# smileyenot983/reconstructor

Measured on AMD Instinct MI355X. Metric: descriptor pair-distances/s + BA LM-iterations/s (1k cams, 100k pts), higher is better.
Workload: dtype f16+f64

## Files before the change

reconstructor_amd/csrc/coarse_i8.h:

```cpp
#pragma once

typedef int i32x16 __attribute__((ext_vector_type(16)));
typedef int i32x4 __attribute__((ext_vector_type(4)));


__device__ __forceinline__ unsigned neg_i8x4(unsigned w)
{
    const unsigned x = ~w;
    return ((x & 0x7F7F7F7Fu) + 0x01010101u) ^ (x & 0x80808080u);
}

template <int ABL, int SH>
__global__ __launch_bounds__(512, 2) void k_coarse_top2_i8(CoarseArgs a)
{
    constexpr int ROWB = 256;
    constexpr int NCB = SH ? 4 : 2;
    constexpr int CW = SH ? 16 : 32;
    constexpr int NKS = SH ? 4 : 8;
    constexpr int CPK = SH ? 4 : 2;
    constexpr int BT = RCN_I8_BT;
    constexpr int TILEB = BT * ROWB;
    constexpr int PIECE = 64 * 16;
    constexpr int NINST = TILEB / 8 / PIECE;
    constexpr int HNP = BT / 64;
    constexpr int NG = NINST + HNP;
    constexpr int BUFB = TILEB + 8 * BT * 4;
    extern __shared__ __attribute__((aligned(16))) char smem[];

    if (!a.sc->coarse_i8) return;
    const int b = blockIdx.x;
    const int item = (b & 7) * a.items_per_xcd + (b >> 3);
    if (item >= a.n_groups * a.tiles_per_pair) return;
    const int grp = item / a.tiles_per_pair, qt = item - grp * a.tiles_per_pair;
    const int2 g = a.groups[grp];
    const int p0 = g.x, R = g.y;
    if (R == 0) return;
    const ImgDev qi = a.imgs[a.pairs[2 * p0]];
    if (qt * RCN_QT >= qi.K) return;

    const int tid = threadIdx.x, lane = tid & 63;
    const int r = SH ? (lane & 15) : (lane & 31), h = SH ? (lane >> 4) : (lane >> 5);
    const int w = __builtin_amdgcn_readfirstlane(tid >> 6);

    i32x4 bq[NCB][NKS];
#pragma unroll
    for (int cb = 0; cb < NCB; ++cb) {
        const int qrow = qt * RCN_QT + w * 64 + cb * CW + r;
        const char *base = reinterpret_cast<const char *>(qi.f16) + (size_t)qrow * ROWB;
        const int sw = qrow & 15;
#pragma unroll
        for (int ks = 0; ks < NKS; ++ks) {
            uint4 v = *reinterpret_cast<const uint4 *>(base + (((ks * CPK + h) ^ sw) << 4));
            v.x = neg_i8x4(v.x); v.y = neg_i8x4(v.y); v.z = neg_i8x4(v.z); v.w = neg_i8x4(v.w);
            bq[cb][ks] = __builtin_bit_cast(i32x4, v);
        }
    }

    struct TrainRec { const char *img; const int *hn; int nT; int pad; };
    static_assert(sizeof(TrainRec) * RCN_GROUP <= RCN_TBL_BYTES, "train-record table does not fit its LDS slot");
    TrainRec *tbl = reinterpret_cast<TrainRec *>(smem + RCN_NBUF * BUFB);
    if (tid < R) {
        const ImgDev ti = a.imgs[a.pairs[2 * (p0 + tid) + 1]];
        TrainRec rec;
        rec.img = reinterpret_cast<const char *>(ti.f16);
        rec.hn = reinterpret_cast<const int *>(ti.hn);
        rec.nT = ti.K >= 2 ? (ti.K + BT - 1) / BT : 0;
        rec.pad = 0;
        tbl[tid] = rec;
    }
    __syncthreads();
    auto tiles_of = [&](int rr) -> int { return __builtin_amdgcn_readfirstlane(tbl[rr].nT); };

    int s_pair = 0, s_tile = 0, s_nT = 0, staged = 0;
    const char *s_timg = nullptr;
    const int *s_hn = nullptr;
    auto s_seek = [&]() {
        while (s_pair < R) {
            s_nT = tiles_of(s_pair);
            if (s_nT > 0) {
                const unsigned long long pf = reinterpret_cast<unsigned long long>(tbl[s_pair].img);
                const unsigned long long ph = reinterpret_cast<unsigned long long>(tbl[s_pair].hn);
                s_timg = reinterpret_cast<const char *>(((unsigned long long)__builtin_amdgcn_readfirstlane((unsigned)(pf >> 32)) << 32) |
                                                        (unsigned)__builtin_amdgcn_readfirstlane((unsigned)pf));
                s_hn = reinterpret_cast<const int *>(((unsigned long long)__builtin_amdgcn_readfirstlane((unsigned)(ph >> 32)) << 32) |
                                                     (unsigned)__builtin_amdgcn_readfirstlane((unsigned)ph));
                s_tile = 0;
                return;
            }
            ++s_pair;
        }
    };
    auto stage_next = [&]() {
        if (s_pair >= R) return;
        char *bbase = smem + (staged % RCN_NBUF) * BUFB;
#pragma unroll
        for (int i = 0; i < NINST; ++i) {
            const int off = (w * NINST + i) * PIECE;
            const char *src = s_timg + (size_t)s_tile * TILEB + off + lane * 16;
            __builtin_amdgcn_global_load_lds(
                (const __attribute__((address_space(1))) void *)src,
                (__attribute__((address_space(3))) void *)(bbase + off), 16, 0, 0);
        }
#pragma unroll
        for (int hp = 0; hp < HNP; ++hp)
            __builtin_amdgcn_global_load_lds(
                (const __attribute__((address_space(1))) void *)(s_hn + s_tile * BT + 64 * hp + lane),
                (__attribute__((address_space(3))) void *)(bbase + TILEB + w * (BT * 4) + 256 * hp), 4, 0, 0);
        ++staged;
        if (++s_tile == s_nT) { ++s_pair; s_seek(); }
    };
    s_seek();
#pragma unroll
    for (int i = 0; i < RCN_PD; ++i) stage_next();

    unsigned m1[NCB], m2[NCB];
    i32x16 pX0, pX1, pY0, pY1;
    i32x4 qX[2][4], qY[2][4];
    auto top2 = [&](int cb, unsigned u) {
        if constexpr ((ABL & 1) != 0) return;
        const unsigned lo = min(m1[cb], m2[cb]), hi = max(m1[cb], m2[cb]);
        m2[cb] = max(lo, min(hi, u));
        m1[cb] = min(m1[cb], u);
    };
    constexpr bool LATE = ((ABL & 32) != 0) != (SH == 0);
    unsigned fk[NCB][3], fs[NCB];
    auto push = [&](int cb, int j, unsigned u) {
        if constexpr ((ABL & 1) != 0) return;
        if constexpr ((ABL & 16) != 0) { top2(cb, u); return; }
        if constexpr (LATE) {
            if ((j & 3) < 3) fk[cb][j & 3] = u;
            else top2_fold4(m1[cb], m2[cb], fk[cb][0], fk[cb][1], fk[cb][2], u);
            return;
        }
        switch (j & 3) {
        case 0: case 2: fk[cb][0] = u; break;
        case 1: fs[cb] = top2_fold_pair(m1[cb], fk[cb][0], u); break;
        default: m2[cb] = umin3(m2[cb], fs[cb], top2_fold_pair(m1[cb], fk[cb][0], u)); break;
        }
    };
    auto key = [&](int acc, unsigned idx) -> unsigned { return ((unsigned)acc << RCN_I8_IDX_BITS) | idx; };
    auto lds_read = [&](unsigned addr) -> u32x4 {
        u32x4 v;
        asm volatile("ds_read_b128 %0, %1" : "=v"(v) : "v"(addr));
        return v;
    };
    auto step = [&](i32x16 &c0, i32x16 &c1, const i32x16 &p0v, const i32x16 &p1v, unsigned tile,
                    unsigned hnl, int rb, unsigned prev_rowbase) {
        if constexpr (SH == 0) {
        const int lrow = rb * 32 + r;
        const unsigned arow = tile + lrow * ROWB;
        const int sw = lrow & 15;
        u32x4 h0, h1, h2, h3, f0, f1;
        h0 = lds_read(hnl + (rb * 32 + 0 + 4 * h) * 4);
        h1 = lds_read(hnl + (rb * 32 + 8 + 4 * h) * 4);
        h2 = lds_read(hnl + (rb * 32 + 16 + 4 * h) * 4);
        h3 = lds_read(hnl + (rb * 32 + 24 + 4 * h) * 4);
        f0 = lds_read(arow + ((h ^ sw) << 4));
        asm volatile("s_waitcnt lgkmcnt(0)" : "+v"(h0), "+v"(h1), "+v"(h2), "+v"(h3), "+v"(f0));
        i32x16 hnv;
        hnv[0] = (int)h0.x; hnv[1] = (int)h0.y; hnv[2] = (int)h0.z; hnv[3] = (int)h0.w;
        hnv[4] = (int)h1.x; hnv[5] = (int)h1.y; hnv[6] = (int)h1.z; hnv[7] = (int)h1.w;
        hnv[8] = (int)h2.x; hnv[9] = (int)h2.y; hnv[10] = (int)h2.z; hnv[11] = (int)h2.w;
        hnv[12] = (int)h3.x; hnv[13] = (int)h3.y; hnv[14] = (int)h3.z; hnv[15] = (int)h3.w;
        auto kstep = [&](int ks, u32x4 &cur, u32x4 &nxt) {
            if (ks > 0) asm volatile("s_waitcnt lgkmcnt(0)" : "+v"(cur), "+v"(c1));
            if (ks + 1 < NKS) nxt = lds_read(arow + ((((ks + 1) * 2 + h) ^ sw) << 4));
            const i32x4 av = __builtin_bit_cast(i32x4, cur);
            c0 = __builtin_amdgcn_mfma_i32_32x32x32_i8(av, bq[0][ks], ks == 0 ? hnv : c0, 0, 0, 0);
#pragma unroll
            for (int reg = ks * 16 / NKS; reg < (ks + 1) * 16 / NKS; ++reg)
                push(0, reg, key(p0v[reg], prev_rowbase + (reg & 3) + 8 * (reg >> 2)));
            c1 = __builtin_amdgcn_mfma_i32_32x32x32_i8(av, bq[1][ks], ks == 0 ? hnv : c1, 0, 0, 0);
#pragma unroll
            for (int reg = ks * 16 / NKS; reg < (ks + 1) * 16 / NKS; ++reg)
                push(1, reg, key(p1v[reg], prev_rowbase + (reg & 3) + 8 * (reg >> 2)));
        };
#pragma unroll
        for (int ks = 0; ks < NKS; ks += 2) {
            kstep(ks, f0, f1);
            kstep(ks + 1, f1, f0);
        }
        }
    };
    auto step16 = [&](i32x4 (&c)[2][4], const i32x4 (&pv)[2][4], unsigned tile, unsigned hnl, int rb, unsigned prev_rowbase) {
        if constexpr (SH == 1) {
            const int lrow = rb * 32 + r;
            const unsigned arow0 = tile + lrow * ROWB, arow1 = arow0 + 16 * ROWB;
            const int sw = lrow & 15;
            u32x4 hA, hB, f0a, f0b, f1a, f1b;
            hA = lds_read(hnl + (rb * 32 + 0 + 4 * h) * 4);
            hB = lds_read(hnl + (rb * 32 + 16 + 4 * h) * 4);
            f0a = lds_read(arow0 + ((h ^ sw) << 4));
            f0b = lds_read(arow1 + ((h ^ sw) << 4));
            asm volatile("s_waitcnt lgkmcnt(0)" : "+v"(hA), "+v"(hB), "+v"(f0a), "+v"(f0b));
            i32x4 hn[2];
            hn[0] = __builtin_bit_cast(i32x4, hA);
            hn[1] = __builtin_bit_cast(i32x4, hB);
            constexpr int EPK = 32 / NKS;
            auto kstep = [&](int ks, u32x4 &ca_, u32x4 &cb_, u32x4 &na_, u32x4 &nb_) {
                if (ks > 0) asm volatile("s_waitcnt lgkmcnt(0)" : "+v"(ca_), "+v"(cb_), "+v"(c[1][3]));
                if (ks + 1 < NKS) {
                    na_ = lds_read(arow0 + ((((ks + 1) * 4 + h) ^ sw) << 4));
                    nb_ = lds_read(arow1 + ((((ks + 1) * 4 + h) ^ sw) << 4));
                }
                const i32x4 av[2] = {__builtin_bit_cast(i32x4, ca_), __builtin_bit_cast(i32x4, cb_)};
#pragma unroll
                for (int m = 0; m < 8; ++m) {
                    const int sh = m >> 2, cb = m & 3;
                    c[sh][cb] = __builtin_amdgcn_mfma_i32_16x16x64_i8(av[sh], bq[cb][ks], ks == 0 ? hn[sh] : c[sh][cb], 0, 0, 0);
#pragma unroll
                    for (int e = ks * EPK + m * EPK / 8; e < ks * EPK + (m + 1) * EPK / 8; ++e) {
                        const int es = e >> 4, ecb = (e >> 2) & 3, er = e & 3;
                        push(ecb, er, key(pv[es][ecb][er], prev_rowbase + 16 * es + er));
                    }
                }
            };
#pragma unroll
            for (int ks = 0; ks < NKS; ks += 2) {
                kstep(ks, f0a, f0b, f1a, f1b);
                kstep(ks + 1, f1a, f1b, f0a, f0b);
            }
        }
    };
    const unsigned smem_base = (unsigned)(size_t)(const __attribute__((address_space(3))) char *)smem;

    int done = 0;
    for (int rr = 0; rr < R; ++rr) {
        const int nT = tiles_of(rr);
        if (nT == 0) continue;
#pragma unroll
        for (int cb = 0; cb < NCB; ++cb) m1[cb] = m2[cb] = 0xFFFFFFFFu;
        if constexpr (SH == 0) {
#pragma unroll
            for (int i = 0; i < 16; ++i) { pY0[i] = RCN_I8_PAD_ACC; pY1[i] = RCN_I8_PAD_ACC; }
        } else {
#pragma unroll
            for (int i = 0; i < 32; ++i) qY[i >> 4][(i >> 2) & 3][i & 3] = RCN_I8_PAD_ACC;
        }
        for (int t = 0; t < nT; ++t, ++done) {
            stage_next();
            const int ahead = staged - done - 1;
            if (ahead >= 2) asm volatile("s_waitcnt vmcnt(%0)" ::"i"(2 * NG) : "memory");
            else if (ahead == 1) asm volatile("s_waitcnt vmcnt(%0)" ::"i"(NG) : "memory");
            else asm volatile("s_waitcnt vmcnt(0)" ::: "memory");
            __builtin_amdgcn_s_barrier();
            const unsigned tile = smem_base + (done % RCN_NBUF) * BUFB;
            const unsigned hnl = tile + TILEB + w * (BT * 4);
            const unsigned base = (unsigned)(t * BT);
#pragma unroll
            for (int rb = 0; rb < BT / 32; rb += 2) {
                if constexpr (SH == 0) {
                    step(pX0, pX1, pY0, pY1, tile, hnl, rb, base + 32u * rb - 32u);
                    step(pY0, pY1, pX0, pX1, tile, hnl, rb + 1, base + 32u * rb);
                } else {
                    step16(qX, qY, tile, hnl, rb, base + 32u * rb - 32u);
                    step16(qY, qX, tile, hnl, rb + 1, base + 32u * rb);
                }
            }
        }
        if (ABL & 1) {
            if constexpr (SH == 0) asm volatile("" ::"v"(pY0), "v"(pY1), "v"(pX0), "v"(pX1));
            else {
#pragma unroll
                for (int i = 0; i < 8; ++i) asm volatile("" ::"v"(qY[i >> 2][i & 3]), "v"(qX[i >> 2][i & 3]));
            }
        }
        {
            const unsigned rowbase = (unsigned)((nT - 1) * BT + BT - 32);
            if constexpr (SH == 0) {
#pragma unroll
                for (int reg = 0; reg < 16; ++reg) {
                    const unsigned idx = rowbase + (reg & 3) + 8 * (reg >> 2);
                    push(0, reg, key(pY0[reg], idx));
                    push(1, reg, key(pY1[reg], idx));
                }
            } else {
#pragma unroll
                for (int e = 0; e < 32; ++e) {
                    const int es = e >> 4, ecb = (e >> 2) & 3, er = e & 3;
                    push(ecb, er, key(qY[es][ecb][er], rowbase + 16 * es + er));
                }
            }
        }
        if constexpr (SH == 0) {
#pragma unroll
            for (int cb = 0; cb < 2; ++cb) {
                unsigned a1 = m1[cb] | (unsigned)(4 * h), a2 = m2[cb] | (unsigned)(4 * h);
                if (m1[cb] == 0xFFFFFFFFu) a1 = 0xFFFFFFFFu;
                if (m2[cb] == 0xFFFFFFFFu) a2 = 0xFFFFFFFFu;
                unsigned b1 = __shfl_xor(a1, 32), b2 = __shfl_xor(a2, 32);
                unsigned r1 = min(a1, b1);
                unsigned r2 = min(max(a1, b1), min(a2, b2));
                const int qrow = qt * RCN_QT + w * 64 + cb * 32 + r;
                if (h == 0 && qrow < qi.K) a.cand[(size_t)(p0 + rr) * a.kq_stride + qrow] = make_uint2(r1, r2);
            }
        } else {
#pragma unroll
            for (int cb = 0; cb < 4; ++cb) {
                unsigned a1 = m1[cb] | (unsigned)(4 * h), a2 = m2[cb] | (unsigned)(4 * h);
                if (m1[cb] == 0xFFFFFFFFu) a1 = 0xFFFFFFFFu;
                if (m2[cb] == 0xFFFFFFFFu) a2 = 0xFFFFFFFFu;
#pragma unroll
                for (int o = 16; o <= 32; o <<= 1) {
                    const unsigned b1 = __shfl_xor(a1, o), b2 = __shfl_xor(a2, o);
                    const unsigned r1 = min(a1, b1);
                    a2 = min(max(a1, b1), min(a2, b2));
                    a1 = r1;
                }
                const int qrow = qt * RCN_QT + w * 64 + cb * 16 + r;
                if (h == 0 && qrow < qi.K) a.cand[(size_t)(p0 + rr) * a.kq_stride + qrow] = make_uint2(a1, a2);
            }
        }
    }
}
```

reconstructor_amd/csrc/match.hip:

```cpp
#include "rcn_internal.h"

#include <algorithm>
#include <cmath>

typedef _Float16 half8 __attribute__((ext_vector_type(8)));
typedef float f32x16 __attribute__((ext_vector_type(16)));
typedef float f32x4 __attribute__((ext_vector_type(4)));
typedef unsigned u32x4 __attribute__((ext_vector_type(4)));

#define RCN_TBL_BYTES ((RCN_GROUP * 24 + 127) / 128 * 128)
#define RCN_NBUF 4
#define RCN_PD 2
#define RCN_CHUNK_ROWS (1ll << 27)
#define RCN_BT 64
#define RCN_PAD_HN 1.0e30f
#define RCN_I8_IDX_MASK ((1u << RCN_I8_IDX_BITS) - 1u)
#define RCN_I8_PAD_ACC ((1 << (32 - RCN_I8_IDX_BITS)) - 1)
#define RCN_I8_BT 128
#define RCN_I8_RES_MAX 8.01
#define RCN_I8_M_MAX 720.0
#define RCN_I8_PEAK_MAX 8.0

template <int DP> __host__ __device__ __forceinline__ int swz(int row)
{
    if (DP >= 128) return row & 15;
    if (DP == 64) return (row >> 1) & 7;
    return (row >> 2) & 3;
}

__device__ __forceinline__ int norm_bin(double n2)
{
    if (!(n2 > 0.0)) return 0;
    if (!(n2 <= 1.7976931348623157e308)) return RCN_HIST_BINS - 1;
    const int e = ilogb(n2) + RCN_HIST_BINS / 2;
    return e < 1 ? 1 : (e > RCN_HIST_BINS - 1 ? RCN_HIST_BINS - 1 : e);
}
template <bool VEC4>
__global__ __launch_bounds__(256) void k_rowstats(const float *__restrict__ x, int K, int D, double *__restrict__ nrm2,
                                                  unsigned *__restrict__ g_maxabs_bits,
                                                  unsigned long long *__restrict__ g_maxnrm2_bits, unsigned *__restrict__ g_hist)
{
    __shared__ unsigned s_hist[RCN_HIST_BINS];
    for (int i = threadIdx.x; i < RCN_HIST_BINS; i += 256) s_hist[i] = 0u;
    __syncthreads();
    const int lane = threadIdx.x & 63;
    const int wave = (blockIdx.x * blockDim.x + threadIdx.x) >> 6, nwaves = (gridDim.x * blockDim.x) >> 6;
    float ma = 0.f;
    double mx = 0.0;
    if (VEC4) {
        const int sub = lane & 15, rsel = lane >> 4, nv = D >> 2;
        for (int j0 = wave * 4; j0 < K; j0 += nwaves * 4) {
            const int j = j0 + rsel;
            double acc = 0.0;
            if (j < K) {
                const float4 *row = reinterpret_cast<const float4 *>(x + (size_t)j * D);
                for (int k = sub; k < nv; k += 16) {
                    const float4 v = row[k];
                    ma = fmaxf(fmaxf(ma, fmaxf(fabsf(v.x), fabsf(v.y))), fmaxf(fabsf(v.z), fabsf(v.w)));
                    acc = fma((double)v.x, (double)v.x, acc);
                    acc = fma((double)v.y, (double)v.y, acc);
                    acc = fma((double)v.z, (double)v.z, acc);
                    acc = fma((double)v.w, (double)v.w, acc);
                }
            }
            for (int o = 8; o; o >>= 1) acc += __shfl_xor(acc, o);
            if (sub == 0 && j < K) { nrm2[j] = acc; atomicAdd(&s_hist[norm_bin(acc)], 1u); }
            mx = fmax(mx, acc);
        }
        for (int o = 32; o >= 16; o >>= 1) mx = fmax(mx, __shfl_xor(mx, o));
    } else {
        for (int j = wave; j < K; j += nwaves) {
            const float *row = x + (size_t)j * D;
            double acc = 0.0;
            for (int k = lane; k < D; k += 64) {
                const float v = row[k];
                ma = fmaxf(ma, fabsf(v));
                acc = fma((double)v, (double)v, acc);
            }
            for (int o = 32; o; o >>= 1) acc += __shfl_xor(acc, o);
            if (lane == 0) { nrm2[j] = acc; atomicAdd(&s_hist[norm_bin(acc)], 1u); }
            mx = fmax(mx, acc);
        }
    }
    __shared__ float s_ma[4];
    __shared__ double s_mx[4];
    for (int o = 32; o; o >>= 1) ma = fmaxf(ma, __shfl_xor(ma, o));
    if (lane == 0) { s_ma[threadIdx.x >> 6] = ma; s_mx[threadIdx.x >> 6] = mx; }
    __syncthreads();
    if (threadIdx.x == 0) {
        for (int w = 1; w < 4; ++w) { ma = fmaxf(ma, s_ma[w]); mx = fmax(mx, s_mx[w]); }
        const unsigned a = __float_as_uint(ma);
        const unsigned long long m = (unsigned long long)__double_as_longlong(mx);
        if (a > __hip_atomic_load(g_maxabs_bits, __ATOMIC_RELAXED, __HIP_MEMORY_SCOPE_AGENT)) atomicMax(g_maxabs_bits, a);
        if (m > __hip_atomic_load(g_maxnrm2_bits, __ATOMIC_RELAXED, __HIP_MEMORY_SCOPE_AGENT)) atomicMax(g_maxnrm2_bits, m);
    }
    for (int i = threadIdx.x; i < RCN_HIST_BINS; i += 256)
        if (s_hist[i]) atomicAdd(g_hist + i, s_hist[i]);
}

__global__ __launch_bounds__(256) void k_norm_hist(const double *__restrict__ nrm2, long n, unsigned *__restrict__ g_hist)
{
    __shared__ unsigned s_hist[RCN_HIST_BINS];
    for (int i = threadIdx.x; i < RCN_HIST_BINS; i += 256) s_hist[i] = 0u;
    __syncthreads();
    for (long i = (long)blockIdx.x * 256 + threadIdx.x; i < n; i += (long)gridDim.x * 256) atomicAdd(&s_hist[norm_bin(nrm2[i])], 1u);
    __syncthreads();
    for (int i = threadIdx.x; i < RCN_HIST_BINS; i += 256)
        if (s_hist[i]) atomicAdd(g_hist + i, s_hist[i]);
}

template <int DP>
__global__ void k_prepare(const float *__restrict__ x, const double *__restrict__ nrm2, int K,
                          int Kp, int D, const ScaleDev *__restrict__ sc,
                          _Float16 *__restrict__ f16, float *__restrict__ hn, unsigned long long *__restrict__ bigmin)
{
    constexpr int CPR = DP / 8;
    if (sc->coarse_i8) return;
    const float scale = sc->sf;
    const double half_s2 = sc->hs2, bias = sc->bias, thr2 = sc->thr2;
    int gid = blockIdx.x * blockDim.x + threadIdx.x;
    int row = gid / CPR, c = gid % CPR;
    if (row >= Kp) return;
    const bool big = row < K && thr2 <= 1.7976931348623157e308 && !(nrm2[row] < thr2);
    half8 v;
    if (big) {
#pragma unroll
        for (int e = 0; e < 8; ++e) v[e] = (_Float16)0.f;
        if (c == 0) atomicMin(bigmin, (unsigned long long)__double_as_longlong(nrm2[row] == nrm2[row] ? nrm2[row] : 0.0));
    } else if (row < K && c * 8 + 8 <= D && (D & 3) == 0) {
        const float4 lo = *reinterpret_cast<const float4 *>(x + (size_t)row * D + c * 8);
        const float4 hi = *reinterpret_cast<const float4 *>(x + (size_t)row * D + c * 8 + 4);
        v[0] = (_Float16)(lo.x * scale); v[1] = (_Float16)(lo.y * scale); v[2] = (_Float16)(lo.z * scale); v[3] = (_Float16)(lo.w * scale);
        v[4] = (_Float16)(hi.x * scale); v[5] = (_Float16)(hi.y * scale); v[6] = (_Float16)(hi.z * scale); v[7] = (_Float16)(hi.w * scale);
    } else {
#pragma unroll
        for (int e = 0; e < 8; ++e) {
            int k = c * 8 + e;
            float f = (row < K && k < D) ? x[(size_t)row * D + k] * scale : 0.f;
            v[e] = (_Float16)f;
        }
    }
    *reinterpret_cast<half8 *>(f16 + (size_t)row * DP + ((c ^ swz<DP>(row)) * 8)) = v;
    if (c == 0) hn[row] = (row < K && !big) ? (float)(half_s2 * nrm2[row] + bias) : RCN_PAD_HN;
}

template <int DP>
__global__ void k_prepare_batch(const float *__restrict__ x, const double *__restrict__ nrm2,
                                int n, int Kslot, int Kp, int D, const ScaleDev *__restrict__ sc,
                                _Float16 *__restrict__ f16, float *__restrict__ hn,
                                const int32_t *__restrict__ Ks, unsigned long long *__restrict__ bigmin)
{
    constexpr int CPR = DP / 8;
    if (sc->coarse_i8) return;
    const float scale = sc->sf;
    const double half_s2 = sc->hs2, bias = sc->bias, thr2 = sc->thr2;
    const long gid = (long)blockIdx.x * blockDim.x + threadIdx.x;
    const long grow = gid / CPR;
    const int c = (int)(gid % CPR);
    if (grow >= (long)n * Kp) return;
    const int img = (int)(grow / Kp), row = (int)(grow % Kp);
    const float *xi = x + (size_t)img * Kslot * D;
    const int K = Ks ? Ks[img] : Kslot;
    const double n2 = row < K ? nrm2[(size_t)img * Kslot + row] : 0.0;
    const bool big = row < K && thr2 <= 1.7976931348623157e308 && !(n2 < thr2);
    half8 v;
    if (big) {
#pragma unroll
        for (int e = 0; e < 8; ++e) v[e] = (_Float16)0.f;
        if (c == 0) atomicMin(bigmin + img, (unsigned long long)__double_as_longlong(n2 == n2 ? n2 : 0.0));
    } else if (row < K && c * 8 + 8 <= D && (D & 3) == 0) {
        const float4 lo = *reinterpret_cast<const float4 *>(xi + (size_t)row * D + c * 8);
// ... 1808 lines not shown
                                                            im.f16, im.hn, im.bigmin);
    if (DP == 256 && ctx->i8_allowed)
        k_prepare_i8<<<(im.Kp * 16 + 255) / 256, 256, 0, ctx->stream>>>(im.f32, im.nrm2, 1, im.K, im.Kp, ctx->D, ctx->scale_dev.as<ScaleDev>(),
                                                                       reinterpret_cast<signed char *>(im.f16), 0L, reinterpret_cast<int *>(im.hn), im.i8n,
                                                                       nullptr, im.bigmin, ctx->counters.as<unsigned>() + RCN_I8_WORD);
}

int rcn_int_resolve_scale(rcn_ctx *ctx)
{
    if (!ctx->scale_on_device) return RCN_OK;
    RCN_HIP(hipMemcpyAsync(&ctx->scale_host, ctx->scale_dev.p, sizeof(ScaleDev), hipMemcpyDeviceToHost, ctx->stream));
    RCN_HIP(rcn_int_stream_wait(ctx));
    ctx->scale = ctx->scale_host.s;
    ctx->bias = ctx->scale_host.bias;
    ctx->max_norm = ctx->scale_host.n_max;
    ctx->thr2 = ctx->scale_host.thr2;
    ctx->coarse_i8_host = ctx->scale_host.coarse_i8;
    ctx->scale_on_device = false;
    return RCN_OK;
}

int rcn_int_i8_commit(rcn_ctx *ctx)
{
    if (!ctx->i8_allowed) return RCN_OK;
    k_i8_commit<<<1, 64, 0, ctx->stream>>>(ctx->counters.as<unsigned>() + RCN_I8_WORD, ctx->scale_dev.as<ScaleDev>());
    RCN_HIP(hipGetLastError());
    return RCN_OK;
}

int rcn_int_prepare_all(rcn_ctx *ctx)
{
    if (ctx->prepared) return RCN_OK;
    RCN_HIP(ctx->scale_dev.reserve(sizeof(ScaleDev)));
    const int DPa = ctx->DP ? ctx->DP : 32;
    bool on_device = ctx->want_dev_scale;
    if (on_device)
        for (const auto &kv : ctx->images) on_device = on_device && kv.second.dirty;
    bool allow_i8 = ctx->DP == 256 && !ctx->coarse_i8_off && !ctx->coarse_w4 && ctx->coarse_shape < 0 && !ctx->force_exact;
    for (const auto &kv : ctx->images) allow_i8 = allow_i8 && kv.second.Kp <= (1 << RCN_I8_IDX_BITS) && kv.second.i8n;
    bool moved = allow_i8 != ctx->i8_allowed;
    ctx->i8_allowed = allow_i8;
    unsigned *i8_max = ctx->counters.as<unsigned>() + RCN_I8_WORD;
    if (on_device) {
        RCN_HIP(hipMemsetAsync(i8_max, 0, 2 * sizeof(unsigned), ctx->stream));
        k_fix_scale<<<1, 64, 0, ctx->stream>>>(ctx->counters.as<unsigned>(), DPa, allow_i8 ? 1 : 0, ctx->scale_dev.as<ScaleDev>());
        RCN_HIP(hipGetLastError());
        ctx->scale_on_device = true;
    } else {
        { int rcs = rcn_int_resolve_scale(ctx); if (rcs) return rcs; }
        {
            long resident = 0;
            for (const auto &kv : ctx->images) resident += kv.second.slab < 0 ? kv.second.K : 0;
            for (const Slab &sl : ctx->slabs) resident += sl.live ? (long)sl.n * sl.K : 0;
            if (ctx->hist_rows > 2 * resident + 1024) {
                unsigned *hist = ctx->counters.as<unsigned>() + RCN_HIST_WORD;
                RCN_HIP(hipMemsetAsync(hist, 0, RCN_HIST_BINS * sizeof(unsigned), ctx->stream));
                for (const auto &kv : ctx->images)
                    if (kv.second.slab < 0 && kv.second.K > 0)
                        k_norm_hist<<<std::min(64, (kv.second.K + 255) / 256), 256, 0, ctx->stream>>>(kv.second.nrm2, kv.second.K, hist);
                for (const Slab &sl : ctx->slabs)
                    if (sl.live) k_norm_hist<<<std::min(1024L, ((long)sl.n * sl.K + 255) / 256), 256, 0, ctx->stream>>>(sl.nrm2, (long)sl.n * sl.K, hist);
                RCN_HIP(hipGetLastError());
                ctx->hist_rows = resident;
            }
        }
        std::vector<unsigned> hc(RCN_HIST_WORD + RCN_HIST_BINS, 0u);
        RCN_HIP(hipMemcpyAsync(hc.data(), ctx->counters.p, RCN_COUNTER_BYTES, hipMemcpyDeviceToHost, ctx->stream));
        RCN_HIP(rcn_int_stream_wait(ctx));
        float maxabs;
        double maxn2;
        memcpy(&maxabs, &hc[0], 4);
        memcpy(&maxn2, &hc[2], 8);
        fix_scale(maxabs, maxn2, hc.data() + RCN_HIST_WORD, DPa, allow_i8 ? 1 : 0, &ctx->scale_host);
        const double s = ctx->scale_host.s, bias = ctx->scale_host.bias;
        moved = moved || s != ctx->scale || bias != ctx->bias || ctx->scale_host.thr2 != ctx->thr2 || ctx->scale_host.coarse_i8 != ctx->coarse_i8_host;
        ctx->coarse_i8_host = ctx->scale_host.coarse_i8;
        if (moved) RCN_HIP(hipMemsetAsync(i8_max, 0, 2 * sizeof(unsigned), ctx->stream));
        ctx->thr2 = ctx->scale_host.thr2;
        ctx->scale = s;
        ctx->max_norm = ctx->scale_host.n_max;
        ctx->bias = bias;
        RCN_HIP(hipMemcpyAsync(ctx->scale_dev.p, &ctx->scale_host, sizeof(ScaleDev), hipMemcpyHostToDevice, ctx->stream));
    }

    std::vector<ImgDev> table;
    table.reserve(ctx->images.size());
    int slot = 0;
    std::vector<char> slab_dirty(ctx->slabs.size(), 0);
    for (auto &kv : ctx->images) {
        ImgHost &im = kv.second;
        im.slot = slot++;
        const bool need = moved || im.dirty;
        if (need && im.slab >= 0) slab_dirty[im.slab] = 1;
        if (ctx->DP && im.slab < 0 && need) {
            switch (ctx->DP) {
            case 32: launch_prepare<32>(ctx, im); break;
            case 64: launch_prepare<64>(ctx, im); break;
            case 128: launch_prepare<128>(ctx, im); break;
            default: launch_prepare<256>(ctx, im); break;
            }
            RCN_HIP(hipGetLastError());
        }
        im.dirty = false;
        table.push_back(ImgDev{im.f32, im.f16, im.hn, im.nrm2, im.bigmin, im.K, im.Kp, im.i8n});
    }
    if (ctx->DP)
        for (size_t si = 0; si < ctx->slabs.size(); ++si) {
            const Slab &sl = ctx->slabs[si];
            if (!sl.live || !slab_dirty[si]) continue;
            switch (ctx->DP) {
            case 32: launch_prepare_batch<32>(ctx, sl); break;
            case 64: launch_prepare_batch<64>(ctx, sl); break;
            case 128: launch_prepare_batch<128>(ctx, sl); break;
            default: launch_prepare_batch<256>(ctx, sl); break;
            }
            RCN_HIP(hipGetLastError());
        }
    { int rci = rcn_int_i8_commit(ctx); if (rci) return rci; }
    const bool same = table.size() == ctx->table_host.size() && ctx->img_table.p &&
                      (table.empty() || memcmp(table.data(), ctx->table_host.data(), table.size() * sizeof(ImgDev)) == 0);
    if (!same) {
        RCN_HIP(rcn_int_stream_wait(ctx));
        ctx->table_host.swap(table);
        RCN_HIP(ctx->img_table.reserve(std::max<size_t>(1, ctx->table_host.size()) * sizeof(ImgDev)));
        if (!ctx->table_host.empty())
            RCN_HIP(hipMemcpyAsync(ctx->img_table.p, ctx->table_host.data(), ctx->table_host.size() * sizeof(ImgDev),
                                   hipMemcpyHostToDevice, ctx->stream));
    }
    ctx->prepared = true;
    return RCN_OK;
}

template <int DP> static hipError_t launch_coarse_w4(rcn_ctx *ctx, const CoarseArgs &ca, int blocks)
{
    const size_t lds = (size_t)RCN_NBUF * (RCN_BT * DP * 2 + 4 * 256) + RCN_TBL_BYTES;
    hipError_t e = hipFuncSetAttribute(reinterpret_cast<const void *>(k_coarse_w4<DP>), hipFuncAttributeMaxDynamicSharedMemorySize, (int)lds);
    if (e != hipSuccess) return e;
    k_coarse_w4<DP><<<blocks, 256, lds, ctx->stream>>>(ca);
    return hipGetLastError();
}

template <int DP, int ABL = 0, int SH = 0> static hipError_t launch_coarse(rcn_ctx *ctx, const CoarseArgs &ca, int blocks)
{
    const size_t lds = (size_t)RCN_NBUF * (coarse_bt(DP) * DP * 2 + 8 * coarse_bt(DP) * 4) + RCN_TBL_BYTES;
    hipError_t e = hipFuncSetAttribute(reinterpret_cast<const void *>(k_coarse_top2<DP, ABL, SH>),
                                       hipFuncAttributeMaxDynamicSharedMemorySize, (int)lds);
    if (e != hipSuccess) return e;
    k_coarse_top2<DP, ABL, SH><<<blocks, 512, lds, ctx->stream>>>(ca);
    return hipGetLastError();
}

template <int ABL, int SH> static hipError_t launch_coarse_i8(rcn_ctx *ctx, const CoarseArgs &ca, int blocks)
{
    const size_t lds = (size_t)RCN_NBUF * (RCN_I8_BT * 256 + 8 * RCN_I8_BT * 4) + RCN_TBL_BYTES;
    hipError_t e = hipFuncSetAttribute(reinterpret_cast<const void *>(k_coarse_top2_i8<ABL, SH>),
                                       hipFuncAttributeMaxDynamicSharedMemorySize, (int)lds);
    if (e != hipSuccess) return e;
    k_coarse_top2_i8<ABL, SH><<<blocks, 512, lds, ctx->stream>>>(ca);
    return hipGetLastError();
}

static int fill_grid_shape(rcn_ctx *ctx, const int32_t *pairs_host, int32_t n_pairs)
{
    grid::GridShape &gs = ctx->grid_shape;
    std::vector<const ImgHost *> flat;
    {
        int32_t lo = INT32_MAX, hi = INT32_MIN;
        for (const auto &kv : ctx->images)
            if (kv.first != INT32_MIN && kv.first != INT32_MIN + 1) { lo = std::min(lo, kv.first); hi = std::max(hi, kv.first); }
        if (lo >= 0 && hi >= lo && hi < (1 << 24)) {
            flat.assign((size_t)hi + 1, nullptr);
            for (const auto &kv : ctx->images)
                if (kv.first >= 0) flat[kv.first] = &kv.second;
        }
    }
    auto lookup = [&](int32_t id) -> const ImgHost * {
        if (!flat.empty() && id >= 0 && (size_t)id < flat.size()) return flat[id];
        auto it = ctx->images.find(id);
        return it == ctx->images.end() ? nullptr : &it->second;
    };
    gs.slots.resize(2 * (size_t)n_pairs); gs.k.resize((size_t)n_pairs);
    for (int p = 0; p < n_pairs; ++p) {
        const ImgHost *a = lookup(pairs_host[2 * p]), *b = lookup(pairs_host[2 * p + 1]);
        if (!a || !b) {
            ctx->set_error("rcn_match_grid: image id not resident");
            return RCN_ERR_NOT_FOUND;
        }
        gs.slots[2 * (size_t)p] = a->slot; gs.slots[2 * (size_t)p + 1] = b->slot;
        gs.k[p] = {a->K, b->K, b->Kp};
    }
    gs.D = ctx->D; gs.DP = ctx->DP;
    gs.n_slots = (int)ctx->table_host.size(); gs.n_cu = ctx->prop.multiProcessorCount;
    gs.chunk_rows = ctx->chunk_rows; gs.mid_rows = ctx->mid_rows;
    gs.i8_allowed = ctx->i8_allowed; gs.force_exact = ctx->force_exact; gs.no_item_order = ctx->no_item_order; gs.mid_i8_off = ctx->mid_i8_off;
    return RCN_OK;
}

static int launch_coarse_stage(rcn_ctx *ctx, const grid::GridPlan &pl, const grid::Chunk &ck, const RerankArgs &ra, uint2 *cand_c)
{
    static_assert(sizeof(grid::Group) == sizeof(int2) && offsetof(grid::Group, count) == offsetof(int2, y), "the arranged groups are uploaded as int2");
    CoarseArgs ca;
    ca.imgs = ra.imgs; ca.pairs = ra.pairs; ca.cand = cand_c;
    ca.groups = ctx->groups_dev.as<int2>() + ck.arr_off;
    ca.n_groups = ck.arr_n; ca.tiles_per_pair = pl.tiles; ca.kq_stride = pl.kq_stride;
    ca.items_per_xcd = ck.items_per_xcd;
    ca.idx_mask = pl.idx_mask;
    ca.sc = ra.sc;
    const int blocks = ca.items_per_xcd * 8;
    hipError_t e;
    if (ctx->coarse_w4 && ctx->DP >= 64) {
        switch (ctx->DP) {
        case 64: e = launch_coarse_w4<64>(ctx, ca, blocks); break;
        case 128: e = launch_coarse_w4<128>(ctx, ca, blocks); break;
        default: e = launch_coarse_w4<256>(ctx, ca, blocks); break;
        }
    } else {
        const int shape = ctx->coarse_shape >= 0 ? ctx->coarse_shape : (ctx->DP == 256 ? 1 : 0);
        if (shape == 1) {
            switch (ctx->DP) {
            case 32: e = launch_coarse<32, 0, 1>(ctx, ca, blocks); break;
            case 64: e = launch_coarse<64, 0, 1>(ctx, ca, blocks); break;
            case 128: e = launch_coarse<128, 0, 1>(ctx, ca, blocks); break;
            default:
#ifdef RCN_DIAG
                switch (ctx->ablate) {
                case 1: e = launch_coarse<256, 1, 1>(ctx, ca, blocks); break;
                case 16: e = launch_coarse<256, 16, 1>(ctx, ca, blocks); break;
                case 9: e = launch_coarse<256, 9, 1>(ctx, ca, blocks); break;
                default: e = launch_coarse<256, 0, 1>(ctx, ca, blocks); break;
                }
#else
                e = launch_coarse<256, 0, 1>(ctx, ca, blocks);
#endif
                break;
            }
        } else {
            switch (ctx->DP) {
            case 32:
#ifdef RCN_DIAG
                if (ctx->ablate == 1) { e = launch_coarse<32, 1, 0>(ctx, ca, blocks); break; }
                if (ctx->ablate == 2) { e = launch_coarse<32, 2, 0>(ctx, ca, blocks); break; }
                if (ctx->ablate == 6) { e = launch_coarse<32, 6, 0>(ctx, ca, blocks); break; }
                if (ctx->ablate == 16) { e = launch_coarse<32, 16, 0>(ctx, ca, blocks); break; }
                if (ctx->ablate == 32) { e = launch_coarse<32, 32, 0>(ctx, ca, blocks); break; }
#endif
                e = launch_coarse<32>(ctx, ca, blocks); break;
            case 64: e = launch_coarse<64>(ctx, ca, blocks); break;
            case 128:
#ifdef RCN_DIAG
                if (ctx->ablate == 1) { e = launch_coarse<128, 1, 0>(ctx, ca, blocks); break; }
                if (ctx->ablate == 2) { e = launch_coarse<128, 2, 0>(ctx, ca, blocks); break; }
                if (ctx->ablate == 6) { e = launch_coarse<128, 6, 0>(ctx, ca, blocks); break; }
                if (ctx->ablate == 16) { e = launch_coarse<128, 16, 0>(ctx, ca, blocks); break; }
                if (ctx->ablate == 32) { e = launch_coarse<128, 32, 0>(ctx, ca, blocks); break; }
#endif
                e = launch_coarse<128>(ctx, ca, blocks); break;
            default: e = launch_coarse<256>(ctx, ca, blocks); break;
            }
        }
    }
    RCN_HIP(e);
    if (ctx->i8_allowed) {
#ifdef RCN_DIAG
        if (ctx->coarse_i8_shape == 0) e = launch_coarse_i8<0, 0>(ctx, ca, blocks);
        else if (ctx->ablate == 1) e = launch_coarse_i8<1, 1>(ctx, ca, blocks);
        else if (ctx->ablate == 16) e = launch_coarse_i8<16, 1>(ctx, ca, blocks);
        else if (ctx->ablate == 32) e = launch_coarse_i8<32, 1>(ctx, ca, blocks);
        else
#endif
        e = launch_coarse_i8<0, 1>(ctx, ca, blocks);
        RCN_HIP(e);
    }
    return RCN_OK;
}

struct MidSource {
    const uint2 *cand;
    const unsigned long long *fb_list;
    const unsigned *fb_count;
    const float *thr_in;
    const unsigned *tacc_in;
    uint32_t midrows;
};

static int launch_mid_tier(rcn_ctx *ctx, const grid::GridPlan &pl, const RerankArgs &ra, unsigned *ccnt, const MidSource &src, bool defer_rows)
{
    const grid::MidLayout &mo = pl.mid_ws;
    const int n_slots = ctx->grid_shape.n_slots, cus = ctx->prop.multiProcessorCount;
    hipStream_t st = ctx->stream;
    char *mw = ctx->mid_ws.as<char>();
    MidArgs ma;
    memset(&ma, 0, sizeof(ma));
    ma.imgs = ra.imgs; ma.pairs = ra.pairs; ma.cand = src.cand; ma.fb_list = src.fb_list; ma.fb_count = src.fb_count;
    ma.thr_in = src.thr_in; ma.tacc_in = src.tacc_in;
    ma.sorted = (unsigned long long *)(mw + mo.sorted); ma.thr = (float *)(mw + mo.thr); ma.ccount = (unsigned *)(mw + mo.cc); ma.tacc = (unsigned *)(mw + mo.tacc);
    ma.clist = (int32_t *)(mw + mo.cl); ma.fb2_list = (unsigned long long *)(mw + mo.fb2);
    ma.hist = (unsigned *)(mw + mo.bins); ma.offs = ma.hist + (n_slots + 1); ma.cursor = ma.offs + (n_slots + 1); ma.ibase = ma.cursor + (n_slots + 1);
    ma.n_items = ccnt + 3; ma.fb2_count = ccnt + 2;
    ma.out = ra.out; ma.out_stride = ra.out_stride; ma.sc = ra.sc; ma.n_slots = n_slots; ma.kq_stride = pl.kq_stride; ma.D = ra.D;
    ma.all_to_fallback = ra.all_to_fallback; ma.idx_mask = pl.idx_mask; ma.ratio = ra.ratio; ma.midrows = src.midrows;
    if (defer_rows) {
        k_mid_defer<<<cus * 2, 256, 0, st>>>(ma, (unsigned long long *)(mw + mo.def), (float *)(mw + mo.defthr), (unsigned *)(mw + mo.deftacc), ccnt, (unsigned)mo.rows_cap);
        k_mid_defer_commit<<<1, 64, 0, st>>>(ccnt, (unsigned)mo.rows_cap);
    }
    k_mid_hist<<<cus * 4, 256, 0, st>>>(ma);
    k_mid_bins<<<1, 1024, 0, st>>>(ma);
    k_mid_scatter<<<cus * 4, 256, 0, st>>>(ma);
// ... 503 lines not shown
```

Before: 5135 billion.

## Share hn staging across waves, precompute LDS addresses, prefetch next row block

The int8 coarse top-2 kernel now stages the per-tile norm vector once per buffer, issued by one rotating wave with 16-byte loads, instead of a copy per wave. This shrinks each LDS ring buffer and drops those loads from the vmcnt wait counts. The SH=1 path precomputes per-lane fragment addresses once and folds row-block offsets into ds_read immediate offsets. It also issues the next row block's first fragment and norm reads during the last k-step of the current block, controlled by RCN_I8_EARLY_OPEN. The trade is more live VGPRs and template-unrolled code, and other waves may now read the shared norm buffer through only the barrier.

```diff
diff --git a/reconstructor_amd/csrc/coarse_i8.h b/reconstructor_amd/csrc/coarse_i8.h
--- a/reconstructor_amd/csrc/coarse_i8.h
+++ b/reconstructor_amd/csrc/coarse_i8.h
@@ -1,8 +1,20 @@
 #pragma once
+
+#include "coarse_i8_addr.h"
 
 typedef int i32x16 __attribute__((ext_vector_type(16)));
 typedef int i32x4 __attribute__((ext_vector_type(4)));
 
+
+template <int V> struct I8Const { static constexpr int value = V; };
+
+template <unsigned IMM> __device__ __forceinline__ u32x4 lds_read_imm(unsigned base)
+{
+    static_assert(IMM < i8addr::OFFSET_LIMIT && IMM % 16 == 0, "offset field");
+    u32x4 v;
+    asm volatile("ds_read_b128 %0, %1 offset:%2" : "=&v"(v) : "v"(base), "n"(IMM));
+    return v;
+}
 
 __device__ __forceinline__ unsigned neg_i8x4(unsigned w)
 {
@@ -22,9 +34,8 @@
     constexpr int TILEB = BT * ROWB;
     constexpr int PIECE = 64 * 16;
     constexpr int NINST = TILEB / 8 / PIECE;
-    constexpr int HNP = BT / 64;
-    constexpr int NG = NINST + HNP;
-    constexpr int BUFB = TILEB + 8 * BT * 4;
+    constexpr int BUFB = i8addr::BUF_BYTES;
+    static_assert(ROWB == i8addr::ROW_BYTES && BT == i8addr::TILE_ROWS && BT * 4 == 32 * 16, "coarse_i8_addr.h describes another tile");
     extern __shared__ __attribute__((aligned(16))) char smem[];
 
     if (!a.sc->coarse_i8) return;
@@ -101,11 +112,10 @@
                 (const __attribute__((address_space(1))) void *)src,
                 (__attribute__((address_space(3))) void *)(bbase + off), 16, 0, 0);
         }
-#pragma unroll
-        for (int hp = 0; hp < HNP; ++hp)
+        if (w == (staged & 7) && lane < 32)
             __builtin_amdgcn_global_load_lds(
-                (const __attribute__((address_space(1))) void *)(s_hn + s_tile * BT + 64 * hp + lane),
-                (__attribute__((address_space(3))) void *)(bbase + TILEB + w * (BT * 4) + 256 * hp), 4, 0, 0);
+                (const __attribute__((address_space(1))) void *)(s_hn + s_tile * BT + 4 * lane),
+                (__attribute__((address_space(3))) void *)(bbase + TILEB), 16, 0, 0);
         ++staged;
         if (++s_tile == s_nT) { ++s_pair; s_seek(); }
     };
@@ -182,26 +192,44 @@
         }
         }
     };
-    auto step16 = [&](i32x4 (&c)[2][4], const i32x4 (&pv)[2][4], unsigned tile, unsigned hnl, int rb, unsigned prev_rowbase) {
+    unsigned fl[4], hl = 0, fb[4], hb = 0;
+    if constexpr (SH == 1) {
+#pragma unroll
+        for (int ks = 0; ks < 4; ++ks) fl[ks] = i8addr::frag_lane((unsigned)r, (unsigned)h, (unsigned)ks);
+        hl = i8addr::hn_lane((unsigned)h);
+        asm volatile("" : "+v"(fl[0]), "+v"(fl[1]), "+v"(fl[2]), "+v"(fl[3]), "+v"(hl));
+    }
+    constexpr bool EARLY = RCN_I8_EARLY_OPEN != 0;
+    auto step16 = [&](auto RB, i32x4 (&c)[2][4], i32x4 (&pv)[2][4], u32x4 (&open)[4], u32x4 (&next)[4], unsigned prev_rowbase) {
         if constexpr (SH == 1) {
-            const int lrow = rb * 32 + r;
-            const unsigned arow0 = tile + lrow * ROWB, arow1 = arow0 + 16 * ROWB;
-            const int sw = lrow & 15;
-            u32x4 hA, hB, f0a, f0b, f1a, f1b;
-            hA = lds_read(hnl + (rb * 32 + 0 + 4 * h) * 4);
-            hB = lds_read(hnl + (rb * 32 + 16 + 4 * h) * 4);
-            f0a = lds_read(arow0 + ((h ^ sw) << 4));
-            f0b = lds_read(arow1 + ((h ^ sw) << 4));
-            asm volatile("s_waitcnt lgkmcnt(0)" : "+v"(hA), "+v"(hB), "+v"(f0a), "+v"(f0b));
+            constexpr int rb = decltype(RB)::value;
+            constexpr bool opened = EARLY && rb > 0;
+            if constexpr (!opened) {
+                open[0] = lds_read_imm<i8addr::hn_imm(rb, 0)>(hb);
+                open[1] = lds_read_imm<i8addr::hn_imm(rb, 1)>(hb);
+                open[2] = lds_read_imm<i8addr::frag_imm(rb, 0)>(fb[0]);
+                open[3] = lds_read_imm<i8addr::frag_imm(rb, 1)>(fb[0]);
+                asm volatile("s_waitcnt lgkmcnt(0)" : "+v"(open[0]), "+v"(open[1]), "+v"(open[2]), "+v"(open[3]));
+            } else {
+                asm volatile("s_waitcnt lgkmcnt(0)" : "+v"(open[0]), "+v"(open[1]), "+v"(open[2]), "+v"(open[3]), "+v"(pv[1][3]));
+            }
             i32x4 hn[2];
-            hn[0] = __builtin_bit_cast(i32x4, hA);
-            hn[1] = __builtin_bit_cast(i32x4, hB);
+            hn[0] = __builtin_bit_cast(i32x4, open[0]);
+            hn[1] = __builtin_bit_cast(i32x4, open[1]);
+            u32x4 &f0a = open[2], &f0b = open[3];
+            u32x4 f1a, f1b;
             constexpr int EPK = 32 / NKS;
-            auto kstep = [&](int ks, u32x4 &ca_, u32x4 &cb_, u32x4 &na_, u32x4 &nb_) {
-                if (ks > 0) asm volatile("s_waitcnt lgkmcnt(0)" : "+v"(ca_), "+v"(cb_), "+v"(c[1][3]));
-                if (ks + 1 < NKS) {
-                    na_ = lds_read(arow0 + ((((ks + 1) * 4 + h) ^ sw) << 4));
-                    nb_ = lds_read(arow1 + ((((ks + 1) * 4 + h) ^ sw) << 4));
+            auto kstep = [&](auto KS, u32x4 &ca_, u32x4 &cb_, u32x4 &na_, u32x4 &nb_) {
+                constexpr int ks = decltype(KS)::value;
+                if constexpr (ks > 0) asm volatile("s_waitcnt lgkmcnt(0)" : "+v"(ca_), "+v"(cb_), "+v"(c[1][3]));
+                if constexpr (ks + 1 < NKS) {
+                    na_ = lds_read_imm<i8addr::frag_imm(rb, 0)>(fb[(ks + 1) & 3]);
+                    nb_ = lds_read_imm<i8addr::frag_imm(rb, 1)>(fb[(ks + 1) & 3]);
+                } else if constexpr (EARLY && rb + 1 < BT / 32) {
+                    next[0] = lds_read_imm<i8addr::hn_imm(rb + 1, 0)>(hb);
+                    next[1] = lds_read_imm<i8addr::hn_imm(rb + 1, 1)>(hb);
+                    next[2] = lds_read_imm<i8addr::frag_imm(rb + 1, 0)>(fb[0]);
+                    next[3] = lds_read_imm<i8addr::frag_imm(rb + 1, 1)>(fb[0]);
                 }
                 const i32x4 av[2] = {__builtin_bit_cast(i32x4, ca_), __builtin_bit_cast(i32x4, cb_)};
 #pragma unroll
@@ -215,11 +243,10 @@
                     }
                 }
             };
-#pragma unroll
-            for (int ks = 0; ks < NKS; ks += 2) {
-                kstep(ks, f0a, f0b, f1a, f1b);
-                kstep(ks + 1, f1a, f1b, f0a, f0b);
-            }
+            kstep(I8Const<0>{}, f0a, f0b, f1a, f1b);
+            kstep(I8Const<1>{}, f1a, f1b, f0a, f0b);
+            kstep(I8Const<2>{}, f0a, f0b, f1a, f1b);
+            kstep(I8Const<3>{}, f1a, f1b, f0a, f0b);
         }
     };
     const unsigned smem_base = (unsigned)(size_t)(const __attribute__((address_space(3))) char *)smem;
@@ -240,22 +267,29 @@
         for (int t = 0; t < nT; ++t, ++done) {
             stage_next();
             const int ahead = staged - done - 1;
-            if (ahead >= 2) asm volatile("s_waitcnt vmcnt(%0)" ::"i"(2 * NG) : "memory");
-            else if (ahead == 1) asm volatile("s_waitcnt vmcnt(%0)" ::"i"(NG) : "memory");
+            if (ahead >= 2) asm volatile("s_waitcnt vmcnt(%0)" ::"i"(2 * NINST) : "memory");
+            else if (ahead == 1) asm volatile("s_waitcnt vmcnt(%0)" ::"i"(NINST) : "memory");
             else asm volatile("s_waitcnt vmcnt(0)" ::: "memory");
             __builtin_amdgcn_s_barrier();
             const unsigned tile = smem_base + (done % RCN_NBUF) * BUFB;
-            const unsigned hnl = tile + TILEB + w * (BT * 4);
             const unsigned base = (unsigned)(t * BT);
-#pragma unroll
-            for (int rb = 0; rb < BT / 32; rb += 2) {
-                if constexpr (SH == 0) {
+            if constexpr (SH == 0) {
+                const unsigned hnl = tile + TILEB;
+#pragma unroll
+                for (int rb = 0; rb < BT / 32; rb += 2) {
                     step(pX0, pX1, pY0, pY1, tile, hnl, rb, base + 32u * rb - 32u);
                     step(pY0, pY1, pX0, pX1, tile, hnl, rb + 1, base + 32u * rb);
-                } else {
-                    step16(qX, qY, tile, hnl, rb, base + 32u * rb - 32u);
-                    step16(qY, qX, tile, hnl, rb + 1, base + 32u * rb);
-                }
+                }
+            } else {
+                static_assert(BT / 32 == 4, "four row blocks per tile are spelled out");
+#pragma unroll
+                for (int ks = 0; ks < 4; ++ks) fb[ks] = tile + fl[ks];
+                hb = tile + hl;
+                u32x4 oA[4], oB[4];
+                step16(I8Const<0>{}, qX, qY, oA, oB, base - 32u);
+                step16(I8Const<1>{}, qY, qX, oB, oA, base);
+                step16(I8Const<2>{}, qX, qY, oA, oB, base + 32u);
+                step16(I8Const<3>{}, qY, qX, oB, oA, base + 64u);
             }
         }
         if (ABL & 1) {
diff --git a/reconstructor_amd/csrc/coarse_i8_addr.h b/reconstructor_amd/csrc/coarse_i8_addr.h
--- /dev/null
+++ b/reconstructor_amd/csrc/coarse_i8_addr.h
@@ -0,0 +1,27 @@
+#pragma once
+
+#if defined(__HIPCC__) || defined(__CUDACC__)
+#define RCN_I8A_FN __host__ __device__ constexpr
+#else
+#define RCN_I8A_FN constexpr
+#endif
+
+namespace i8addr {
+
+constexpr unsigned ROW_BYTES = 256;
+constexpr unsigned TILE_ROWS = 128;
+constexpr unsigned TILE_BYTES = TILE_ROWS * ROW_BYTES;
+constexpr unsigned HN_BYTES = TILE_ROWS * 4;
+constexpr unsigned BUF_BYTES = TILE_BYTES + HN_BYTES;
+constexpr unsigned OFFSET_LIMIT = 1u << 16;
+
+RCN_I8A_FN unsigned frag_lane(unsigned r, unsigned h, unsigned ks) { return r * ROW_BYTES + (((4u * ks + h) ^ r) << 4); }
+RCN_I8A_FN unsigned frag_imm(unsigned rb, unsigned half) { return (32u * rb + 16u * half) * ROW_BYTES; }
+RCN_I8A_FN unsigned hn_lane(unsigned h) { return 16u * h; }
+RCN_I8A_FN unsigned hn_imm(unsigned rb, unsigned half) { return TILE_BYTES + (32u * rb + 16u * half) * 4u; }
+RCN_I8A_FN unsigned buffer_base(unsigned buf) { return buf * BUF_BYTES; }
+
+static_assert(BUF_BYTES % 16 == 0, "ring buffers stay 16-byte aligned");
+static_assert(frag_imm(3, 1) < OFFSET_LIMIT && hn_imm(3, 1) < OFFSET_LIMIT, "an immediate does not fit the offset field");
+
+}
diff --git a/reconstructor_amd/csrc/match.hip b/reconstructor_amd/csrc/match.hip
--- a/reconstructor_amd/csrc/match.hip
+++ b/reconstructor_amd/csrc/match.hip
@@ -17,6 +17,9 @@
 #define RCN_I8_IDX_MASK ((1u << RCN_I8_IDX_BITS) - 1u)
 #define RCN_I8_PAD_ACC ((1 << (32 - RCN_I8_IDX_BITS)) - 1)
 #define RCN_I8_BT 128
+#ifndef RCN_I8_EARLY_OPEN
+#define RCN_I8_EARLY_OPEN 1
+#endif
 #define RCN_I8_RES_MAX 8.01
 #define RCN_I8_M_MAX 720.0
 #define RCN_I8_PEAK_MAX 8.0
@@ -2131,7 +2134,7 @@
 
 template <int ABL, int SH> static hipError_t launch_coarse_i8(rcn_ctx *ctx, const CoarseArgs &ca, int blocks)
 {
-    const size_t lds = (size_t)RCN_NBUF * (RCN_I8_BT * 256 + 8 * RCN_I8_BT * 4) + RCN_TBL_BYTES;
+    const size_t lds = (size_t)RCN_NBUF * i8addr::BUF_BYTES + RCN_TBL_BYTES;
     hipError_t e = hipFuncSetAttribute(reinterpret_cast<const void *>(k_coarse_top2_i8<ABL, SH>),
                                        hipFuncAttributeMaxDynamicSharedMemorySize, (int)lds);
     if (e != hipSuccess) return e;
```

Measured after the change: 5394 billion, median of 6. +5.0%, better.
